# kyle-wedgwood/ArmadilloCUDALinearInterpolation

Measured on AMD Instinct MI355X. Metric: interpolated points/sec (fp64), higher is better.
Workload: dtype f64; 1 GPU; 1D linear interp, 1e+08 random queries on 1e+06-point grid, fp64 (BASELINE configs[1]); queries_per_gpu=100000000, grid_nodes=1000000, table=general, table_mode=0, table_bytes=8000008, entry_point=mi_interp1_f64_dev, query_set=every rank its own set of 100000000 queries

## Files before the change

### armadillocudalinearinterpolation_amd/_lib.py

```python
import ctypes as C
import os

from . import _build

_lib = None


class MiError(RuntimeError):
    def __init__(self, code, msg):
        super().__init__("libmi355interp error %d: %s" % (code, msg))
        self.code = code


class EdmParams(C.Structure):
    _fields_ = [
        ("vth", C.c_float), ("a1", C.c_float), ("a2", C.c_float), ("b1", C.c_float), ("b2", C.c_float),
        ("I", C.c_float), ("L", C.c_float),
        ("newton_tol", C.c_double),
        ("newton_max_iter", C.c_uint32),
        ("n_spikes", C.c_uint32),
        ("time_horizon", C.c_float),
        ("n_grid", C.c_uint32),
        ("n_real", C.c_uint32),
        ("beta_mean", C.c_float),
        ("beta_stddev", C.c_float),
        ("seed", C.c_uint64),
        ("math_mode", C.c_int),
        ("mean_quirk", C.c_int),
        ("max_events", C.c_uint32),
        ("real_offset", C.c_uint32),
        ("dedup_identical", C.c_uint32),
    ]


_vp, _sz, _dbl, _i32, _u32, _f32 = C.c_void_p, C.c_size_t, C.c_double, C.c_int, C.c_uint32, C.c_float
_pp = C.POINTER(C.c_void_p)

SIGNATURES = {
    "mi_abi_version": (_i32, []),
    "mi_debug_pinned_ranges": (_sz, []),
    "mi_debug_sweep_ds_launches": (_sz, []),
    "mi_debug_sweep_ds_launches_base": (_sz, []),
    "mi_debug_interp1_phased_sweep": (_i32, [_vp, _vp, _vp, _vp, _sz, _dbl, _i32, _i32]),
    "mi_debug_each_launches": (_sz, [_i32]),
    "mi_debug_slices2_launches": (_sz, [_i32]),
    "mi_debug_rows1_launches": (_sz, [_i32]),
    "mi_debug_rowpairs_launches": (_sz, [_i32]),
    "mi_debug_nearest_launches": (_sz, [_i32]),
    "mi_debug_nearest_batched_launches": (_sz, [_i32]),
    "mi_debug_grid1_formula": (_i32, [_vp, C.POINTER(_i32), C.POINTER(_i32)]),
    "mi_last_error": (C.c_char_p, [_vp]),
    "mi_ctx_create": (_i32, [_i32, _pp]),
    "mi_ctx_destroy": (_i32, [_vp]),
    "mi_ctx_set_stream": (_i32, [_vp, _vp]),
    "mi_ctx_own_stream": (_i32, [_vp]),
    "mi_ctx_synchronize": (_i32, [_vp]),
    "mi_ctx_set_query_order": (_i32, [_vp, _i32]),
    "mi_ctx_device_info": (_i32, [_vp, C.c_char_p, _sz, C.POINTER(_i32), C.POINTER(_sz)]),
    "mi_timer_create": (_i32, [_vp, _pp]),
    "mi_timer_destroy": (_i32, [_vp]),
    "mi_timer_start": (_i32, [_vp]),
    "mi_timer_stop": (_i32, [_vp]),
    "mi_timer_elapsed_ms": (_i32, [_vp, C.POINTER(_f32)]),
    "mi_grid1_create": (_i32, [_vp, _vp, _vp, _sz, C.c_uint, _pp]),
    "mi_grid1_create_uniform": (_i32, [_vp, _dbl, _dbl, _vp, _sz, C.c_uint, _pp]),
    "mi_grid1_destroy": (_i32, [_vp]),
    "mi_grid1_info": (_i32, [_vp, C.POINTER(_sz), C.POINTER(_i32), C.POINTER(_sz)]),
    "mi_interp1_f64_dev": (_i32, [_vp, _vp, _vp, _vp, _sz, _dbl]),
    "mi_interp1_f64_dev_v2": (_i32, [_vp, _vp, _vp, _vp, _sz, _dbl]),
    "mi_interp1_f64_dev_v2_base": (_i32, [_vp, _vp, _vp, _vp, _sz, _dbl]),
    "mi_interp1_f64_host": (_i32, [_vp, _vp, _vp, _vp, _sz, _dbl]),
    "mi_interp1_f64": (_i32, [_vp, _vp, _vp, _sz, _vp, _vp, _sz, _dbl]),
    "mi_interp1_nearest_f64_dev": (_i32, [_vp, _vp, _vp, _vp, _sz, _dbl]),
    "mi_interp1_nearest_f64_host": (_i32, [_vp, _vp, _vp, _vp, _sz, _dbl]),
    "mi_interp1_nearest_f64": (_i32, [_vp, _vp, _vp, _sz, _vp, _vp, _sz, _dbl]),
    "mi_grid2_create": (_i32, [_vp, _vp, _sz, _vp, _sz, _vp, C.c_uint, _pp]),
    "mi_grid2_create_uniform": (_i32, [_vp, _dbl, _dbl, _sz, _dbl, _dbl, _sz, _vp, C.c_uint, _pp]),
    "mi_grid2_destroy": (_i32, [_vp]),
    "mi_grid2_info": (_i32, [_vp, C.POINTER(_sz)]),
    "mi_interp2_f64_dev": (_i32, [_vp, _vp, _vp, _vp, _vp, _sz, _dbl]),
    "mi_interp2_f64_host": (_i32, [_vp, _vp, _vp, _vp, _vp, _sz, _dbl]),
    "mi_interp2_grid_f64_dev": (_i32, [_vp, _vp, _vp, _sz, _vp, _sz, _vp, _dbl]),
    "mi_interp2_grid_f64_host": (_i32, [_vp, _vp, _vp, _sz, _vp, _sz, _vp, _dbl]),
    "mi_axis1_create": (_i32, [_vp, _vp, _sz, C.c_uint, _pp]),
    "mi_axis1_create_uniform": (_i32, [_vp, _dbl, _dbl, _sz, _pp]),
    "mi_axis1_destroy": (_i32, [_vp]),
    "mi_interp1_cols_f64_dev": (_i32, [_vp, _vp, _vp, _sz, _sz, _vp, _sz, _vp, _sz, _dbl]),
    "mi_interp1_cols_f64_host": (_i32, [_vp, _vp, _vp, _sz, _sz, _vp, _sz, _vp, _sz, _dbl]),
    "mi_interp1_cols_nearest_f64_dev": (_i32, [_vp, _vp, _vp, _sz, _sz, _vp, _sz, _vp, _sz, _dbl]),
    "mi_interp1_pairs_f64_dev": (_i32, [_vp, _vp, _sz, _vp, _sz, _sz, _vp, _sz, _vp, _sz, _vp, _sz, _dbl, _vp]),
    "mi_interp1_pairs_f64_host": (_i32, [_vp, _vp, _sz, _vp, _sz, _sz, _vp, _sz, _vp, _sz, _vp, _sz, _dbl, _vp]),
    "mi_interp1_pairs_nearest_f64_dev": (_i32, [_vp, _vp, _sz, _vp, _sz, _sz, _vp, _sz, _vp, _sz, _vp, _sz, _dbl, _vp]),
    "mi_interp1_each_f64_dev": (_i32, [_vp, _vp, _sz, _vp, _sz, _sz, _vp, _sz, _vp, _sz, _sz, _vp, _sz, _dbl, _vp]),
    "mi_interp1_each_f64_host": (_i32, [_vp, _vp, _sz, _vp, _sz, _sz, _vp, _sz, _vp, _sz, _sz, _vp, _sz, _dbl, _vp]),
    "mi_interp2_slices_f64_dev": (_i32, [_vp, _vp, _vp, _vp, _sz, _sz, _sz, _vp, _sz, _vp, _sz, _vp, _sz, _sz, _dbl]),
    "mi_interp1_rows_f64_dev": (_i32, [_vp, _vp, _vp, _sz, _sz, _vp, _sz, _vp, _sz, _dbl]),
# ... 91 lines not shown
```

### armadillocudalinearinterpolation_amd/csrc/mi_sweep_phase.hip

```cpp
#include <algorithm>
#include <atomic>
#include <cmath>
#include <cstdlib>

#include "mi_interp1_sweep.hpp"

using namespace mi_interp1;

namespace {

constexpr unsigned kTilePeriodNs = 27000;
constexpr unsigned kMaxPeriodNs = 1000000;
constexpr int kPhaseWaitPolls = 4096;
constexpr int kPhasesDefault = 4;

template <int FORMULA, int DEFER>
__global__ __launch_bounds__(kPipeThreads) void interp1_phased_sweep_kernel(G1Dev g, const double* __restrict__ xq,
                                                                            double* __restrict__ yq, size_t ntiles,
                                                                            double extrap, double bscale,
                                                                            const int* __restrict__ order_flag,
                                                                            size_t tail, ProbeArgs probe,
                                                                            unsigned phase_shift, unsigned class_ticks)
{
    constexpr int kVec = kSweepK / 2;
    static_assert(DEFER > 0 && DEFER <= kVec, "DEFER counts result vectors of a lane");
    constexpr int kNow = kVec - DEFER;
    constexpr int kHeld = 2 * DEFER;
    __shared__ double sq[kSweepTile];
    __shared__ unsigned hist[2][kSweepBins];
    __shared__ unsigned gbar[2];
    if (*order_flag != 0) return;
    if (threadIdx.x < 2) gbar[threadIdx.x] = 0;
    const int tid = threadIdx.x & (kPipeGroup - 1);
    const int grp = threadIdx.x >> 9;
    const unsigned nwg = gridDim.x;
    const unsigned phases = 1u << phase_shift;
    const unsigned cls = blockIdx.x & (phases - 1);
    unsigned rank = blockIdx.x >> phase_shift;
    for (unsigned k = 0; k < cls; ++k) rank += nwg > k ? (nwg - k + phases - 1) >> phase_shift : 0;
    const bool last_wg = rank == nwg - 1;
    if (probe.host_mailbox && last_wg && threadIdx.x >= kPipeThreads - 64) order_probe_wave(probe);
    const long nloc = ntiles > rank ? (long)((ntiles - rank + nwg - 1) / nwg) : 0;
    if (cls != 0) {
        const unsigned long long t0 = wall_clock64(), want = (unsigned long long)cls * class_ticks;
        for (int poll = 0; poll < kPhaseWaitPolls && wall_clock64() - t0 < want; ++poll) __builtin_amdgcn_s_sleep(8);
    }
    double q[kSweepK];
    double held[kHeld];
    unsigned sp2[kSweepK / 2];
    auto drop_held = [&]() {
#pragma unroll
        for (int u = 0; u < kHeld; ++u) held[u] = 0.0;
    };
    drop_held();
    const unsigned lane_bytes = (unsigned)tid * (unsigned)sizeof(d2);
    auto vec_at = [&](const double* base, long it, int u) {
        const char* row = reinterpret_cast<const char*>(base + ((size_t)rank + (size_t)it * nwg) * kSweepTile) +
                          (size_t)u * kPipeGroup * sizeof(d2);
        return reinterpret_cast<d2*>(const_cast<char*>(row + lane_bytes));
    };
    auto load_tile = [&](long it) {
#pragma unroll
        for (int u = 0; u < kVec; ++u) {
            const d2 v = stream_load(vec_at(xq, it, u));
            q[2 * u] = v.x;
            q[2 * u + 1] = v.y;
        }
    };
    auto store_now = [&](long it) {
#pragma unroll
        for (int u = 0; u < kNow; ++u) {
            d2 v;
            v.x = q[2 * u];
            v.y = q[2 * u + 1];
            stream_store(v, vec_at(yq, it, u));
        }
    };
    auto store_held = [&](long it) {
        if (it < 0) return;
#pragma unroll
        for (int u = 0; u < DEFER; ++u) {
            d2 v;
            v.x = held[2 * u];
            v.y = held[2 * u + 1];
            stream_store(v, vec_at(yq, it, kNow + u));
        }
    };
    for (int b = threadIdx.x; b < 2 * kSweepBins; b += kPipeThreads) (&hist[0][0])[b] = 0;
    if (grp == 0 && nloc > 0) load_tile(0);
    pipe_barrier();
    unsigned* const myhist = hist[grp];
    unsigned gb_target = 0;
    auto group_barrier = [&]() {
        gb_target += kPipeGroup / 64;
        asm volatile("s_waitcnt lgkmcnt(0)" ::: "memory");
        if ((threadIdx.x & 63) == 0) atomicAdd(&gbar[grp], 1u);
        while (*(lds_vu32*)&gbar[grp] < gb_target) __builtin_amdgcn_s_sleep(2);
        asm volatile("" ::: "memory");
    };
    auto gather_step = [&](long it) {
        const bool act = it >= 0;
        const bool rev = (it & 1) != 0;
        const int stride = rev ? -kPipeGroup : kPipeGroup;
        int first = rev ? kSweepTile - 1 - tid : tid;
        if (act) {
#pragma unroll 1
            for (int iv = 0; iv < 4; ++iv) {
                pipe_gather_rounds<0, FORMULA>(g, sq, first, stride, extrap);
                first += 8 * stride;
            }
        }
        pipe_barrier();
        if (act) {
#pragma unroll
            for (int u = 0; u < kSweepK; u += 2) {
                const double a = sq[sp2[u / 2] & 0xffffu], b = sq[sp2[u / 2] >> 16];
                if (u / 2 < kNow) {
                    q[u] = a;
                    q[u + 1] = b;
                } else {
                    held[u - 2 * kNow] = a;
                    held[u + 1 - 2 * kNow] = b;
                }
                if ((u & 6) == 6) __builtin_amdgcn_sched_barrier(0);
            }
        } else {
#pragma unroll
            for (int u = 0; u < kSweepK; ++u) q[u] = 0.0;
            drop_held();
        }
        pipe_barrier();
        if (act) store_now(it);
        __builtin_amdgcn_sched_barrier(0);
        if (it + 2 < nloc) {
            load_tile(it + 2);
        } else {
#pragma unroll
            for (int u = 0; u < kSweepK; ++u) q[u] = 0.0;
        }
        pipe_barrier();
    };
    auto prep_step = [&](long it) {
        const bool act = it + 1 < nloc;
        store_held(it - 1);
        drop_held();
        unsigned rank2[kSweepK / 2];
#pragma unroll
        for (int u = 0; u < kSweepK / 2; ++u) rank2[u] = 0;
        if (act) {
#pragma unroll
            for (int u = 0; u < kSweepK; u += 2) {
                const unsigned r0 = atomicAdd(&myhist[sweep_bin(q[u], g.xmin, bscale)], 1u);
                const unsigned r1 = atomicAdd(&myhist[sweep_bin(q[u + 1], g.xmin, bscale)], 1u);
                rank2[u / 2] = r0 | (r1 << 16);
                if ((u & 6) == 6) __builtin_amdgcn_sched_barrier(0);
            }
            group_barrier();
            if (tid < 64) sweep_prefix_wave(myhist, tid);
            group_barrier();
#pragma unroll
            for (int u = 0; u < kSweepK; u += 2) {
                double qa = q[u], qb = q[u + 1];
                asm volatile("" : "+v"(qa), "+v"(qb));
                const unsigned p0 = myhist[sweep_bin(qa, g.xmin, bscale)] + (rank2[u / 2] & 0xffffu);
                const unsigned p1 = myhist[sweep_bin(qb, g.xmin, bscale)] + (rank2[u / 2] >> 16);
                sp2[u / 2] = p0 | (p1 << 16);
                if ((u & 6) == 6) __builtin_amdgcn_sched_barrier(0);
            }
        } else {
#pragma unroll
            for (int u = 0; u < kSweepK / 2; ++u) sp2[u] = 0;
        }
        pipe_barrier();
        if (act) {
            for (int b = tid; b < kSweepBins; b += kPipeGroup) myhist[b] = 0;
        }
        pipe_barrier();
        if (act) {
#pragma unroll
            for (int u = 0; u < kSweepK; u += 2) {
                sq[sp2[u / 2] & 0xffffu] = q[u];
                sq[sp2[u / 2] >> 16] = q[u + 1];
                if ((u & 6) == 6) __builtin_amdgcn_sched_barrier(0);
            }
        }
        pipe_barrier();
    };
    if (grp == 0) {
        for (long it = -1;;) {
            prep_step(it);
            if (++it >= nloc) break;
            gather_step(it);
            if (++it >= nloc) break;
        }
    } else {
        for (long it = -1;;) {
            gather_step(it);
            if (++it >= nloc) break;
            prep_step(it);
            if (++it >= nloc) break;
        }
    }
    if (nloc > 0 && grp == (int)((nloc - 1) & 1)) store_held(nloc - 1);
    if (tail && last_wg && grp == 0) pipe_tail<0, FORMULA>(g, xq + ntiles * kSweepTile, yq + ntiles * kSweepTile, tail, tid, extrap);
}

struct PhaseEnv {
    int phases;
    unsigned period_ns;
    bool family_hooks;
};
const PhaseEnv& phase_env()
{
    static const PhaseEnv e = [] {
        PhaseEnv v{kPhasesDefault, kTilePeriodNs, false};
        if (const char* s = getenv("MI_SWEEP_XCD_PHASES")) {
            char* end = nullptr;
            const long p = strtol(s, &end, 10);
            if (end != s && (p == 0 || p == 1 || p == 2 || p == 4 || p == 8)) v.phases = (int)p;
            if (end != s && *end == ':') {
                const long ns = strtol(end + 1, nullptr, 10);
                if (ns >= 0 && ns <= (long)kMaxPeriodNs) v.period_ns = (unsigned)ns;
            }
        }
        v.family_hooks = getenv("MI_SWEEP_MIN_BYTES") || getenv("MI_SWEEP_MIN_TILES_PER_CU") || getenv("MI_SWEEP_VARIANT") ||
                         getenv("MI_SWEEP_DEFER");
        return v;
    }();
    return e;
}

std::atomic<size_t> g_phased_launches{0};

unsigned class_ticks(const mi_ctx* ctx, unsigned period_ns, int phases)
{
    int khz = 0;
    if (hipDeviceGetAttribute(&khz, hipDeviceAttributeWallClockRate, ctx->device) != hipSuccess || khz <= 0) khz = 100000;
    return (unsigned)((double)period_ns * (double)khz * 1e-6 / (double)phases);
}

template <int FORMULA>
mi_status launch_phased(mi_ctx* ctx, const G1Dev& d, const double* xq, double* yq, size_t nq, double extrap, int phases,
                        unsigned period_ns, unsigned max_wg, const ProbeArgs& probe)
{
    const size_t ntiles = nq / kSweepTile, head = ntiles * kSweepTile;
    const double bscale = (double)kSweepBins / (d.xmax - d.xmin);
    const int* flags = reinterpret_cast<const int*>(static_cast<const char*>(ctx->reduce_ws) + mi_ctx::kFlagOffset);
    const unsigned cus = (unsigned)(ctx->compute_units > 0 ? ctx->compute_units : 256);
    const unsigned grid = (unsigned)std::max<size_t>(1, std::min<size_t>(ntiles, (size_t)std::min(cus, max_wg)));
    hipLaunchKernelGGL((interp1_phased_sweep_kernel<FORMULA, kSweepDefer(0)>), dim3(grid), dim3(kPipeThreads), 0, ctx->stream, d,
                       xq, yq, ntiles, extrap, bscale, flags, nq - head, probe, (unsigned)(phases == 8 ? 3 : phases == 4 ? 2 : phases == 2 ? 1 : 0),
                       class_ticks(ctx, period_ns, phases));
    MI_LAUNCH_CHECK(ctx, "interp1 phased region-sweep kernel");
    g_phased_launches.fetch_add(1, std::memory_order_relaxed);
    return MI_OK;
}

mi_status launch_phased_formula(mi_ctx* ctx, const G1Dev& d, const double* xq, double* yq, size_t nq, double extrap, int phases,
                                unsigned period_ns, unsigned max_wg, const ProbeArgs& probe)
{
    if (d.formula == 1) return launch_phased<1>(ctx, d, xq, yq, nq, extrap, phases, period_ns, max_wg, probe);
    if (d.formula == 2) return launch_phased<2>(ctx, d, xq, yq, nq, extrap, phases, period_ns, max_wg, probe);
    if (d.formula == 3) return launch_phased<3>(ctx, d, xq, yq, nq, extrap, phases, period_ns, max_wg, probe);
    return launch_phased<0>(ctx, d, xq, yq, nq, extrap, phases, period_ns, max_wg, probe);
}

bool aligned16(const double* xq, const double* yq)
{
    return ((reinterpret_cast<uintptr_t>(xq) | reinterpret_cast<uintptr_t>(yq)) & 15u) == 0;
}

bool span_ok(const G1Dev& d) { return std::isfinite(d.xmax - d.xmin) && (d.xmax - d.xmin) > 0.0; }

}

extern "C" {

size_t mi_debug_sweep_ds_launches(void)
{
    return mi_debug_sweep_ds_launches_base() + g_phased_launches.load(std::memory_order_relaxed);
}

mi_status mi_interp1_f64_dev_v2(mi_ctx* ctx, const mi_grid1* g, const double* xq, double* yq, size_t nq, double extrap)
{
    const PhaseEnv& e = phase_env();
    bool take = e.phases != 0 && !e.family_hooks && ctx && g && xq && yq && g->mode == 0 && aligned16(xq, yq) &&
                g->table_bytes >= ((size_t)5 << 20) && span_ok(g->d) && ctx->query_order != MI_QUERIES_ORDERED;
    if (take) {
        const size_t cus = (size_t)(ctx->compute_units > 0 ? ctx->compute_units : 256);
        take = nq / kSweepTile >= cus * 16;
    }
    ProbeArgs probe{};
    if (take && ctx->query_order == MI_QUERIES_AUTO) {
        take = *reinterpret_cast<volatile int*>(ctx->probe_host) == 0;
        probe = ProbeArgs{xq, nq, g->d.xmin, (double)kSweepBins / (g->d.xmax - g->d.xmin), nullptr, ctx->probe_host_dev};
    }
    if (!take) return mi_interp1_f64_dev_v2_base(ctx, g, xq, yq, nq, extrap);
    MI_HIP(ctx, hipSetDevice(ctx->device));
    return launch_phased_formula(ctx, g->d, xq, yq, nq, extrap, e.phases, e.period_ns, ~0u, probe);
}

mi_status mi_debug_interp1_phased_sweep(mi_ctx* ctx, const mi_grid1* g, const double* xq, double* yq, size_t nq, double extrap,
                                        int phases, int max_workgroups)
{
    MI_REQUIRE(ctx, ctx && g, "mi_debug_interp1_phased_sweep: NULL context or grid");
    MI_REQUIRE(ctx, g->mode == 0 && span_ok(g->d), "mi_debug_interp1_phased_sweep: closed-form tables (mode 0) of positive finite span only");
    MI_REQUIRE(ctx, phases == 1 || phases == 2 || phases == 4 || phases == 8, "mi_debug_interp1_phased_sweep: phases=%d is not 1, 2, 4 or 8", phases);
    MI_REQUIRE(ctx, max_workgroups >= 1, "mi_debug_interp1_phased_sweep: max_workgroups=%d", max_workgroups);
    if (nq == 0) return MI_OK;
    MI_REQUIRE(ctx, xq && yq && aligned16(xq, yq), "mi_debug_interp1_phased_sweep: pointers must be non-NULL and 16-byte aligned");
    MI_HIP(ctx, hipSetDevice(ctx->device));
    ProbeArgs probe{};
    if (ctx->query_order == MI_QUERIES_AUTO && nq >= 4098)
        probe = ProbeArgs{xq, nq, g->d.xmin, (double)kSweepBins / (g->d.xmax - g->d.xmin), nullptr, ctx->probe_host_dev};
    return launch_phased_formula(ctx, g->d, xq, yq, nq, extrap, phases, phase_env().period_ns, (unsigned)max_workgroups, probe);
}

}
```

### include/mi355_interp.h

```cpp
#ifndef MI355_INTERP_H
#define MI355_INTERP_H

#include <stddef.h>
#include <stdint.h>

#ifdef __cplusplus
extern "C" {
#endif

#define MI355_INTERP_ABI_VERSION 4

typedef int mi_status;
enum {
    MI_OK = 0,
    MI_ERR_INVALID_ARG = 1,
    MI_ERR_GRID = 2,
    MI_ERR_HIP = 3,
    MI_ERR_NOMEM = 4,
    MI_ERR_NO_DEVICE = 5
};

typedef struct mi_ctx mi_ctx;
typedef struct mi_grid1 mi_grid1;
typedef struct mi_grid2 mi_grid2;
typedef struct mi_axis1 mi_axis1;
typedef struct mi_edm mi_edm;
typedef struct mi_timer mi_timer;

mi_status mi_ctx_create(int device, mi_ctx** out);
mi_status mi_ctx_destroy(mi_ctx* ctx);
mi_status mi_ctx_set_stream(mi_ctx* ctx, void* stream);
mi_status mi_ctx_own_stream(mi_ctx* ctx);
mi_status mi_ctx_synchronize(mi_ctx* ctx);
const char* mi_last_error(const mi_ctx* ctx);
int mi_abi_version(void);
size_t mi_debug_pinned_ranges(void);
size_t mi_debug_sweep_ds_launches(void);
size_t mi_debug_sweep_ds_launches_base(void);
size_t mi_debug_each_launches(int form);
size_t mi_debug_slices2_launches(int form);
size_t mi_debug_rows1_launches(int form);
size_t mi_debug_rowpairs_launches(int form);
size_t mi_debug_nearest_launches(int form);
size_t mi_debug_nearest_batched_launches(int form);
mi_status mi_debug_grid1_formula(const mi_grid1* g, int* formula, int* pin_last);
#define MI_QUERIES_AUTO    0
#define MI_QUERIES_RANDOM  1
#define MI_QUERIES_ORDERED 2
mi_status mi_ctx_set_query_order(mi_ctx* ctx, int order);
mi_status mi_ctx_device_info(mi_ctx* ctx, char* name, size_t name_len, int* compute_units,
                             size_t* hbm_bytes);

mi_status mi_timer_create(mi_ctx* ctx, mi_timer** out);
mi_status mi_timer_destroy(mi_timer* t);
mi_status mi_timer_start(mi_timer* t);
mi_status mi_timer_stop(mi_timer* t);
mi_status mi_timer_elapsed_ms(mi_timer* t, float* ms);

#define MI_GRID_SANITISE     0x1u
#define MI_GRID_DEVICE_PTRS  0x2u
mi_status mi_grid1_create(mi_ctx* ctx, const double* x, const double* y, size_t n,
                          unsigned flags, mi_grid1** out);
mi_status mi_grid1_create_uniform(mi_ctx* ctx, double x0, double dx, const double* y, size_t n,
                                  unsigned flags, mi_grid1** out);
mi_status mi_grid1_destroy(mi_grid1* g);
mi_status mi_grid1_info(const mi_grid1* g, size_t* n_nodes, int* mode, size_t* table_bytes);

mi_status mi_interp1_f64_dev(mi_ctx* ctx, const mi_grid1* g, const double* xq_dev, double* yq_dev,
                             size_t nq, double extrap_val);
mi_status mi_interp1_f64_dev_v2(mi_ctx* ctx, const mi_grid1* g, const double* xq_dev, double* yq_dev,
                                size_t nq, double extrap_val);
mi_status mi_interp1_f64_dev_v2_base(mi_ctx* ctx, const mi_grid1* g, const double* xq_dev, double* yq_dev,
                                     size_t nq, double extrap_val);
mi_status mi_debug_interp1_phased_sweep(mi_ctx* ctx, const mi_grid1* g, const double* xq_dev, double* yq_dev,
                                        size_t nq, double extrap_val, int phases, int max_workgroups);
mi_status mi_interp1_f64_host(mi_ctx* ctx, const mi_grid1* g, const double* xq, double* yq,
                              size_t nq, double extrap_val);
mi_status mi_interp1_f64(mi_ctx* ctx, const double* x, const double* y, size_t n, const double* xq,
                         double* yq, size_t nq, double extrap_val);

mi_status mi_interp1_nearest_f64_dev(mi_ctx* ctx, const mi_grid1* g, const double* xq_dev, double* yq_dev,
                                     size_t nq, double extrap_val);
mi_status mi_interp1_nearest_f64_host(mi_ctx* ctx, const mi_grid1* g, const double* xq, double* yq,
                                      size_t nq, double extrap_val);
mi_status mi_interp1_nearest_f64(mi_ctx* ctx, const double* x, const double* y, size_t n, const double* xq,
                                 double* yq, size_t nq, double extrap_val);

#define MI_GRID2_COMPACT 0x4u
mi_status mi_grid2_create(mi_ctx* ctx, const double* x, size_t nx, const double* y, size_t ny,
                          const double* z, unsigned flags, mi_grid2** out);
mi_status mi_grid2_create_uniform(mi_ctx* ctx, double x0, double dx, size_t nx, double y0, double dy,
                                  size_t ny, const double* z, unsigned flags, mi_grid2** out);
mi_status mi_grid2_destroy(mi_grid2* g);
mi_status mi_grid2_info(const mi_grid2* g, size_t* table_bytes);
mi_status mi_interp2_f64_dev(mi_ctx* ctx, const mi_grid2* g, const double* xq_dev,
                             const double* yq_dev, double* zq_dev, size_t nq, double extrap_val);
mi_status mi_interp2_f64_host(mi_ctx* ctx, const mi_grid2* g, const double* xq, const double* yq,
                              double* zq, size_t nq, double extrap_val);
mi_status mi_interp2_grid_f64_dev(mi_ctx* ctx, const mi_grid2* g, const double* xi_dev, size_t nxi,
                                  const double* yi_dev, size_t nyi, double* zi_dev, double extrap_val);
mi_status mi_interp2_grid_f64_host(mi_ctx* ctx, const mi_grid2* g, const double* xi, size_t nxi,
                                   const double* yi, size_t nyi, double* zi, double extrap_val);

mi_status mi_axis1_create(mi_ctx* ctx, const double* x, size_t n, unsigned flags, mi_axis1** out);
mi_status mi_axis1_create_uniform(mi_ctx* ctx, double x0, double dx, size_t n, mi_axis1** out);
mi_status mi_axis1_destroy(mi_axis1* axis);
mi_status mi_interp1_cols_f64_dev(mi_ctx* ctx, const mi_axis1* axis, const double* y_dev, size_t ldy, size_t ncols,
                                  const double* xi_dev, size_t nxi, double* yi_dev, size_t ldyi, double extrap_val);
mi_status mi_interp1_cols_f64_host(mi_ctx* ctx, const mi_axis1* axis, const double* y, size_t ldy, size_t ncols,
                                   const double* xi, size_t nxi, double* yi, size_t ldyi, double extrap_val);
mi_status mi_interp1_cols_nearest_f64_dev(mi_ctx* ctx, const mi_axis1* axis, const double* y_dev, size_t ldy, size_t ncols,
                                          const double* xi_dev, size_t nxi, double* yi_dev, size_t ldyi, double extrap_val);

mi_status mi_interp1_pairs_f64_dev(mi_ctx* ctx, const double* x_dev, size_t ldx, const double* y_dev, size_t ldy, size_t n,
                                   const uint32_t* len_dev, size_t ncols, const double* xi_dev, size_t nxi,
                                   double* yi_dev, size_t ldyi, double extrap_val, uint32_t* col_ok_dev);
mi_status mi_interp1_pairs_f64_host(mi_ctx* ctx, const double* x, size_t ldx, const double* y, size_t ldy, size_t n,
                                    const uint32_t* len, size_t ncols, const double* xi, size_t nxi, double* yi,
                                    size_t ldyi, double extrap_val, uint32_t* col_ok);
mi_status mi_interp1_pairs_nearest_f64_dev(mi_ctx* ctx, const double* x_dev, size_t ldx, const double* y_dev, size_t ldy,
                                           size_t n, const uint32_t* len_dev, size_t ncols, const double* xi_dev,
                                           size_t nxi, double* yi_dev, size_t ldyi, double extrap_val,
                                           uint32_t* col_ok_dev);

mi_status mi_interp1_each_f64_dev(mi_ctx* ctx, const double* x_dev, size_t ldx, const double* y_dev, size_t ldy, size_t n,
                                  const uint32_t* len_dev, size_t ncols, const double* xi_dev, size_t ldxi, size_t nxi,
                                  double* yi_dev, size_t ldyi, double extrap_val, uint32_t* col_ok_dev);
mi_status mi_interp1_each_f64_host(mi_ctx* ctx, const double* x, size_t ldx, const double* y, size_t ldy, size_t n,
// ... 134 lines not shown
```

Measured before the change: 164.5 billion points/s.

## Stagger phase classes with partial first tiles instead of clock waits

Splits the phased sweep's work into quarter-tile units and gives each phase class a first tile of a different size (1..4 units). This staggers when workgroups hit the memory-heavy phases without spinning on the wall clock. A partition function balances the remaining units across workgroups and handles partial last tiles. It also adds optional timestamp recording and debug entry points, at the cost of more index arithmetic and 32-bit query counting limits.

```diff
diff --git a/armadillocudalinearinterpolation_amd/_lib.py b/armadillocudalinearinterpolation_amd/_lib.py
--- a/armadillocudalinearinterpolation_amd/_lib.py
+++ b/armadillocudalinearinterpolation_amd/_lib.py
@@ -42,6 +42,8 @@
     "mi_debug_sweep_ds_launches": (_sz, []),
     "mi_debug_sweep_ds_launches_base": (_sz, []),
     "mi_debug_interp1_phased_sweep": (_i32, [_vp, _vp, _vp, _vp, _sz, _dbl, _i32, _i32]),
+    "mi_debug_interp1_phased_sweep_ex": (_i32, [_vp, _vp, _vp, _vp, _sz, _dbl, _i32, _i32, _u32, _vp, _u32]),
+    "mi_debug_sweep_partition": (_i32, [_sz, _u32, _i32, _u32, _u32] + [C.POINTER(_u32)] * 3 + [C.POINTER(_sz)] * 6),
     "mi_debug_each_launches": (_sz, [_i32]),
     "mi_debug_slices2_launches": (_sz, [_i32]),
     "mi_debug_rows1_launches": (_sz, [_i32]),
diff --git a/armadillocudalinearinterpolation_amd/csrc/mi_sweep_partition.hpp b/armadillocudalinearinterpolation_amd/csrc/mi_sweep_partition.hpp
--- /dev/null
+++ b/armadillocudalinearinterpolation_amd/csrc/mi_sweep_partition.hpp
@@ -0,0 +1,115 @@
+#pragma once
+#include <cstddef>
+
+namespace mi_sweep {
+
+constexpr unsigned kUnitQueries = 4096;
+constexpr unsigned kTileUnits = 4;
+constexpr unsigned kMaxPhases = 8;
+
+template <class I>
+struct PartitionT {
+    unsigned ntiles;
+    unsigned first_units;
+    unsigned last_units;
+    I work;
+    I first_start;
+    I mid_origin;
+    I mid_step;
+    I pen_start;
+    I last_start;
+};
+using Partition = PartitionT<size_t>;
+
+__host__ __device__ inline unsigned pack_first_units(unsigned decimal, unsigned P)
+{
+    if (P == 0 || P > kMaxPhases) return 0;
+    unsigned nibbles = 0;
+    for (unsigned k = P; k-- > 0;) {
+        const unsigned digit = decimal % 10u;
+        decimal /= 10u;
+        if (digit < 1 || digit > kTileUnits) return 0;
+        nibbles |= digit << (4 * k);
+    }
+    return decimal == 0 ? nibbles : 0;
+}
+__host__ __device__ inline unsigned first_units_of(unsigned nibbles, unsigned k) { return (nibbles >> (4 * k)) & 15u; }
+
+__host__ __device__ inline unsigned class_size(unsigned nwg, unsigned P, unsigned k) { return nwg > k ? (nwg - k + P - 1) / P : 0; }
+
+namespace detail {
+
+template <class I>
+struct Sums {
+    I first, row1, row2;
+};
+
+template <class I>
+__host__ __device__ inline I min_sz(I a, I b) { return a < b ? a : b; }
+
+template <class I>
+__host__ __device__ inline Sums<I> sums_below(unsigned upto, unsigned nwg, unsigned P, unsigned fu, I w, unsigned rem, I R)
+{
+    Sums<I> s{0, 0, 0};
+    unsigned a = 0;
+    for (unsigned k = 0; k < P; ++k) {
+        const unsigned b = a + class_size(nwg, P, k), hi = b < upto ? b : upto;
+        if (hi > a) {
+            const unsigned n1 = rem > a ? (rem < hi ? rem - a : hi - a) : 0;
+            for (unsigned more = 0; more < 2; ++more) {
+                const I cnt = more ? n1 : hi - a - n1;
+                if (cnt == 0) continue;
+                const I share = w + more, f = min_sz<I>(first_units_of(fu, k), share), left = share - f - kTileUnits * R;
+                s.first += cnt * f;
+                s.row1 += cnt * min_sz<I>(left, kTileUnits);
+                s.row2 += cnt * (left > kTileUnits ? left - kTileUnits : 0);
+            }
+        }
+        a = b;
+    }
+    return s;
+}
+
+}
+
+template <class I>
+__host__ __device__ inline PartitionT<I> sweep_partition(I U, unsigned nwg, unsigned P, unsigned first_units, unsigned rank)
+{
+    PartitionT<I> p{};
+    if (nwg == 0 || rank >= nwg || P == 0 || P > kMaxPhases) return p;
+    const I w = U / nwg;
+    const unsigned rem = (unsigned)(U % nwg);
+    I least = ~(I)0;
+    unsigned a = 0, cls = 0;
+    for (unsigned k = 0; k < P; ++k) {
+        const unsigned b = a + class_size(nwg, P, k);
+        if (b > a) {
+            if (rem > a) least = detail::min_sz<I>(least, w + 1 - detail::min_sz<I>(first_units_of(first_units, k), w + 1));
+            if (rem < b) least = detail::min_sz<I>(least, w - detail::min_sz<I>(first_units_of(first_units, k), w));
+            if (rank >= a && rank < b) cls = k;
+        }
+        a = b;
+    }
+    const I R = least / kTileUnits;
+    const detail::Sums<I> all = detail::sums_below<I>(nwg, nwg, P, first_units, w, rem, R);
+    const detail::Sums<I> low = detail::sums_below<I>(rank, nwg, P, first_units, w, rem, R);
+    p.work = w + (rank < rem ? 1 : 0);
+    const I f = detail::min_sz<I>(first_units_of(first_units, cls), p.work), left = p.work - f - kTileUnits * R;
+    const unsigned t1 = (unsigned)detail::min_sz<I>(left, kTileUnits), t2 = left > kTileUnits ? (unsigned)(left - kTileUnits) : 0;
+    p.first_units = (unsigned)f;
+    p.first_start = low.first;
+    p.mid_origin = all.first + (I)kTileUnits * rank;
+    p.mid_step = (I)kTileUnits * nwg;
+    if (f == 0) return p;
+    const I row1 = all.first + p.mid_step * R + low.row1, row2 = all.first + p.mid_step * R + all.row1 + low.row2;
+    const I ntiles = 1 + R + (t1 ? 1 : 0) + (t2 ? 1 : 0);
+    p.ntiles = (unsigned)ntiles;
+    auto start_of = [&](I i) { return i == 0 ? p.first_start : i <= R ? p.mid_origin + (i - 1) * p.mid_step : i == R + 1 ? row1 : row2; };
+    auto units_of = [&](I i) { return i == 0 ? (unsigned)f : i <= R ? kTileUnits : i == R + 1 ? t1 : t2; };
+    p.last_start = start_of(ntiles - 1);
+    p.last_units = units_of(ntiles - 1);
+    p.pen_start = ntiles >= 2 ? start_of(ntiles - 2) : p.first_start;
+    return p;
+}
+
+}
diff --git a/armadillocudalinearinterpolation_amd/csrc/mi_sweep_phase.hip b/armadillocudalinearinterpolation_amd/csrc/mi_sweep_phase.hip
--- a/armadillocudalinearinterpolation_amd/csrc/mi_sweep_phase.hip
+++ b/armadillocudalinearinterpolation_amd/csrc/mi_sweep_phase.hip
@@ -2,8 +2,10 @@
 #include <atomic>
 #include <cmath>
 #include <cstdlib>
+#include <type_traits>
 
 #include "mi_interp1_sweep.hpp"
+#include "mi_sweep_partition.hpp"
 
 using namespace mi_interp1;
 
@@ -13,23 +15,47 @@
 constexpr unsigned kMaxPeriodNs = 1000000;
 constexpr int kPhaseWaitPolls = 4096;
 constexpr int kPhasesDefault = 4;
-
-template <int FORMULA, int DEFER>
+constexpr size_t kMaxQueries = (size_t)1 << 43;
+constexpr unsigned kFirstUnits4 = 1234;
+constexpr unsigned kFirstUnits2 = 0;
+
+template <int J>
+using unit_c = std::integral_constant<int, J>;
+template <class Body, class Skip>
+__device__ __forceinline__ void for_units(unsigned nu, Body&& body, Skip&& skip)
+{
+    if (nu > 0) body(unit_c<0>{}); else skip(unit_c<0>{});
+    if (nu > 1) body(unit_c<1>{}); else skip(unit_c<1>{});
+    if (nu > 2) body(unit_c<2>{}); else skip(unit_c<2>{});
+    if (nu > 3) body(unit_c<3>{}); else skip(unit_c<3>{});
+}
+
+template <int FORMULA, int DEFER, bool STAMP>
 __global__ __launch_bounds__(kPipeThreads) void interp1_phased_sweep_kernel(G1Dev g, const double* __restrict__ xq,
-                                                                            double* __restrict__ yq, size_t ntiles,
+                                                                            double* __restrict__ yq, size_t nq,
                                                                             double extrap, double bscale,
                                                                             const int* __restrict__ order_flag,
-                                                                            size_t tail, ProbeArgs probe,
-                                                                            unsigned phase_shift, unsigned class_ticks)
+                                                                            ProbeArgs probe, unsigned phase_shift,
+                                                                            unsigned class_ticks, unsigned first_units,
+                                                                            unsigned long long* __restrict__ stamps,
+                                                                            unsigned stamp_cap)
 {
     constexpr int kVec = kSweepK / 2;
+    constexpr int kUnitVec = kVec / (int)mi_sweep::kTileUnits;
     static_assert(DEFER > 0 && DEFER <= kVec, "DEFER counts result vectors of a lane");
+    static_assert(kSweepTile == (int)(mi_sweep::kTileUnits * mi_sweep::kUnitQueries) && kUnitVec == 4, "a unit is a quarter of a tile");
     constexpr int kNow = kVec - DEFER;
     constexpr int kHeld = 2 * DEFER;
     __shared__ double sq[kSweepTile];
     __shared__ unsigned hist[2][kSweepBins];
     __shared__ unsigned gbar[2];
     if (*order_flag != 0) return;
+    auto stamp = [&](unsigned slot) __attribute__((always_inline)) {
+        if constexpr (STAMP) {
+            if (slot < stamp_cap) stamps[(size_t)blockIdx.x * stamp_cap + slot] = wall_clock64();
+        }
+    };
+    if (threadIdx.x == 0) stamp(0);
     if (threadIdx.x < 2) gbar[threadIdx.x] = 0;
     const int tid = threadIdx.x & (kPipeGroup - 1);
     const int grp = threadIdx.x >> 9;
@@ -39,91 +65,155 @@
     unsigned rank = blockIdx.x >> phase_shift;
     for (unsigned k = 0; k < cls; ++k) rank += nwg > k ? (nwg - k + phases - 1) >> phase_shift : 0;
     const bool last_wg = rank == nwg - 1;
-    if (probe.host_mailbox && last_wg && threadIdx.x >= kPipeThreads - 64) order_probe_wave(probe);
-    const long nloc = ntiles > rank ? (long)((ntiles - rank + nwg - 1) / nwg) : 0;
-    if (cls != 0) {
+    auto scalar = [](unsigned v) __attribute__((always_inline)) { return (unsigned)__builtin_amdgcn_readfirstlane((int)v); };
+    const unsigned step = mi_sweep::kTileUnits * nwg;
+    unsigned ntl, org, nus = mi_sweep::kTileUnits | (mi_sweep::kTileUnits << 4), d_first = 0, d_pen = 0, d_last = 0;
+    if (first_units == 0) {
+        const unsigned ntiles = (unsigned)(nq / kSweepTile);
+        ntl = scalar(ntiles > rank ? (ntiles - rank + nwg - 1) / nwg : 0);
+        org = mi_sweep::kTileUnits * rank + step;
+    } else {
+        const mi_sweep::PartitionT<unsigned> part =
+            mi_sweep::sweep_partition<unsigned>((unsigned)(nq / mi_sweep::kUnitQueries), nwg, phases, first_units, rank);
+        ntl = scalar(part.ntiles);
+        nus = scalar(part.first_units | (part.last_units << 4));
+        org = scalar(part.mid_origin);
+        d_first = scalar(part.first_start - (part.mid_origin - step));
+        if (part.ntiles >= 2) d_last = scalar(part.last_start - (part.mid_origin + (part.ntiles - 2) * step));
+        if (part.ntiles >= 3) d_pen = scalar(part.pen_start - (part.mid_origin + (part.ntiles - 3) * step));
+    }
+    const long nloc = (long)ntl;
+    const unsigned k_org = org, k_nus = nus, k_first = d_first, k_pen = d_pen, k_last = d_last;
+    auto tile_units = [scalar, ntl, k_nus](long it) __attribute__((always_inline)) {
+        const unsigned i = scalar((unsigned)it);
+        return i == 0 ? k_nus & 15u : i == ntl - 1 ? k_nus >> 4 : mi_sweep::kTileUnits;
+    };
+    auto tile_at = [scalar, ntl, step, k_org, k_first, k_pen, k_last](long it) __attribute__((always_inline)) {
+        const unsigned i = scalar((unsigned)it);
+        const unsigned fix = i == 0 ? k_first : i == ntl - 1 ? k_last : i == ntl - 2 ? k_pen : 0u;
+        return k_org + (i - 1u) * step + fix;
+    };
+    if (cls != 0 && class_ticks != 0) {
         const unsigned long long t0 = wall_clock64(), want = (unsigned long long)cls * class_ticks;
         for (int poll = 0; poll < kPhaseWaitPolls && wall_clock64() - t0 < want; ++poll) __builtin_amdgcn_s_sleep(8);
     }
     double q[kSweepK];
     double held[kHeld];
     unsigned sp2[kSweepK / 2];
-    auto drop_held = [&]() {
+    auto drop_held = [&]() __attribute__((always_inline)) {
 #pragma unroll
         for (int u = 0; u < kHeld; ++u) held[u] = 0.0;
     };
     drop_held();
     const unsigned lane_bytes = (unsigned)tid * (unsigned)sizeof(d2);
-    auto vec_at = [&](const double* base, long it, int u) {
-        const char* row = reinterpret_cast<const char*>(base + ((size_t)rank + (size_t)it * nwg) * kSweepTile) +
-                          (size_t)u * kPipeGroup * sizeof(d2);
-        return reinterpret_cast<d2*>(const_cast<char*>(row + lane_bytes));
-    };
-    auto load_tile = [&](long it) {
-#pragma unroll
-        for (int u = 0; u < kVec; ++u) {
-            const d2 v = stream_load(vec_at(xq, it, u));
-            q[2 * u] = v.x;
-            q[2 * u + 1] = v.y;
-        }
-    };
-    auto store_now = [&](long it) {
-#pragma unroll
-        for (int u = 0; u < kNow; ++u) {
-            d2 v;
-            v.x = q[2 * u];
-            v.y = q[2 * u + 1];
-            stream_store(v, vec_at(yq, it, u));
-        }
-    };
-    auto store_held = [&](long it) {
+    auto vec_at = [&](const double* base, long it, int u) __attribute__((always_inline)) {
+        const char* row = reinterpret_cast<const char*>(base + (size_t)tile_at(it) * mi_sweep::kUnitQueries);
+        asm("" : "+s"(row));
+        return reinterpret_cast<d2*>(const_cast<char*>(row + (size_t)u * kPipeGroup * sizeof(d2) + lane_bytes));
+    };
+    auto load_tile = [&](long it) __attribute__((always_inline)) {
+        for_units(tile_units(it),
+                  [&](auto j) __attribute__((always_inline)) {
+                      constexpr int J = decltype(j)::value;
+#pragma unroll
+                      for (int u = kUnitVec * J; u < kUnitVec * (J + 1); ++u) {
+                          const d2 v = stream_load(vec_at(xq, it, u));
+                          q[2 * u] = v.x;
+                          q[2 * u + 1] = v.y;
+                      }
+                  },
+                  [&](auto j) __attribute__((always_inline)) {
+                      constexpr int J = decltype(j)::value;
+#pragma unroll
+                      for (int u = 2 * kUnitVec * J; u < 2 * kUnitVec * (J + 1); ++u) q[u] = 0.0;
+                  });
+    };
+    auto store_now = [&](long it) __attribute__((always_inline)) {
+        for_units(tile_units(it),
+                  [&](auto j) __attribute__((always_inline)) {
+                      constexpr int J = decltype(j)::value;
+#pragma unroll
+                      for (int u = kUnitVec * J; u < kUnitVec * (J + 1); ++u) {
+                          if (u < kNow) {
+                              d2 v;
+                              v.x = q[2 * u];
+                              v.y = q[2 * u + 1];
+                              stream_store(v, vec_at(yq, it, u));
+                          }
+                      }
+                  },
+                  [&](auto) __attribute__((always_inline)) {});
+    };
+    auto store_held = [&](long it) __attribute__((always_inline)) {
         if (it < 0) return;
-#pragma unroll
-        for (int u = 0; u < DEFER; ++u) {
-            d2 v;
-            v.x = held[2 * u];
-            v.y = held[2 * u + 1];
-            stream_store(v, vec_at(yq, it, kNow + u));
-        }
+        for_units(tile_units(it),
+                  [&](auto j) __attribute__((always_inline)) {
+                      constexpr int J = decltype(j)::value;
+#pragma unroll
+                      for (int u = kUnitVec * J; u < kUnitVec * (J + 1); ++u) {
+                          if (u >= kNow) {
+                              d2 v;
+                              v.x = held[2 * (u - kNow)];
+                              v.y = held[2 * (u - kNow) + 1];
+                              stream_store(v, vec_at(yq, it, u));
+                          }
+                      }
+                  },
+                  [&](auto) __attribute__((always_inline)) {});
     };
     for (int b = threadIdx.x; b < 2 * kSweepBins; b += kPipeThreads) (&hist[0][0])[b] = 0;
     if (grp == 0 && nloc > 0) load_tile(0);
     pipe_barrier();
+    if (probe.host_mailbox && last_wg && threadIdx.x >= kPipeThreads - 64) order_probe_wave(probe);
     unsigned* const myhist = hist[grp];
     unsigned gb_target = 0;
-    auto group_barrier = [&]() {
+    auto group_barrier = [&]() __attribute__((always_inline)) {
         gb_target += kPipeGroup / 64;
         asm volatile("s_waitcnt lgkmcnt(0)" ::: "memory");
         if ((threadIdx.x & 63) == 0) atomicAdd(&gbar[grp], 1u);
         while (*(lds_vu32*)&gbar[grp] < gb_target) __builtin_amdgcn_s_sleep(2);
         asm volatile("" ::: "memory");
     };
-    auto gather_step = [&](long it) {
+    auto gather_step = [&](long it) __attribute__((always_inline)) {
         const bool act = it >= 0;
+        const unsigned nu = act ? tile_units(it) : 0;
         const bool rev = (it & 1) != 0;
         const int stride = rev ? -kPipeGroup : kPipeGroup;
-        int first = rev ? kSweepTile - 1 - tid : tid;
+        int first = rev ? (int)(nu * mi_sweep::kUnitQueries) - 1 - tid : tid;
         if (act) {
+            if (tid == 0) stamp(1u + (unsigned)it);
 #pragma unroll 1
-            for (int iv = 0; iv < 4; ++iv) {
+            for (int iv = 0; iv < (int)nu; ++iv) {
                 pipe_gather_rounds<0, FORMULA>(g, sq, first, stride, extrap);
                 first += 8 * stride;
             }
         }
         pipe_barrier();
         if (act) {
-#pragma unroll
-            for (int u = 0; u < kSweepK; u += 2) {
-                const double a = sq[sp2[u / 2] & 0xffffu], b = sq[sp2[u / 2] >> 16];
-                if (u / 2 < kNow) {
-                    q[u] = a;
-                    q[u + 1] = b;
-                } else {
-                    held[u - 2 * kNow] = a;
-                    held[u + 1 - 2 * kNow] = b;
-                }
-                if ((u & 6) == 6) __builtin_amdgcn_sched_barrier(0);
-            }
+            for_units(nu,
+                      [&](auto j) __attribute__((always_inline)) {
+                      constexpr int J = decltype(j)::value;
+#pragma unroll
+                          for (int u = 8 * J; u < 8 * (J + 1); u += 2) {
+                              const double a = sq[sp2[u / 2] & 0xffffu], b = sq[sp2[u / 2] >> 16];
+                              if (u / 2 < kNow) {
+                                  q[u] = a;
+                                  q[u + 1] = b;
+                              } else {
+                                  held[u - 2 * kNow] = a;
+                                  held[u + 1 - 2 * kNow] = b;
+                              }
+                          }
+                          __builtin_amdgcn_sched_barrier(0);
+                      },
+                      [&](auto j) __attribute__((always_inline)) {
+                      constexpr int J = decltype(j)::value;
+#pragma unroll
+                          for (int u = 8 * J; u < 8 * (J + 1); ++u) {
+                              if (u / 2 < kNow) q[u] = 0.0;
+                              else held[u - 2 * kNow] = 0.0;
+                          }
+                      });
         } else {
 #pragma unroll
             for (int u = 0; u < kSweepK; ++u) q[u] = 0.0;
@@ -140,33 +230,48 @@
         }
         pipe_barrier();
     };
-    auto prep_step = [&](long it) {
+    auto prep_step = [&](long it) __attribute__((always_inline)) {
         const bool act = it + 1 < nloc;
+        const unsigned nu = act ? tile_units(it + 1) : 0;
         store_held(it - 1);
         drop_held();
         unsigned rank2[kSweepK / 2];
 #pragma unroll
         for (int u = 0; u < kSweepK / 2; ++u) rank2[u] = 0;
         if (act) {
-#pragma unroll
-            for (int u = 0; u < kSweepK; u += 2) {
-                const unsigned r0 = atomicAdd(&myhist[sweep_bin(q[u], g.xmin, bscale)], 1u);
-                const unsigned r1 = atomicAdd(&myhist[sweep_bin(q[u + 1], g.xmin, bscale)], 1u);
-                rank2[u / 2] = r0 | (r1 << 16);
-                if ((u & 6) == 6) __builtin_amdgcn_sched_barrier(0);
-            }
+            for_units(nu,
+                      [&](auto j) __attribute__((always_inline)) {
+                      constexpr int J = decltype(j)::value;
+#pragma unroll
+                          for (int u = 8 * J; u < 8 * (J + 1); u += 2) {
+                              const unsigned r0 = atomicAdd(&myhist[sweep_bin(q[u], g.xmin, bscale)], 1u);
+                              const unsigned r1 = atomicAdd(&myhist[sweep_bin(q[u + 1], g.xmin, bscale)], 1u);
+                              rank2[u / 2] = r0 | (r1 << 16);
+                          }
+                          __builtin_amdgcn_sched_barrier(0);
+                      },
+                      [&](auto) __attribute__((always_inline)) {});
             group_barrier();
             if (tid < 64) sweep_prefix_wave(myhist, tid);
             group_barrier();
-#pragma unroll
-            for (int u = 0; u < kSweepK; u += 2) {
-                double qa = q[u], qb = q[u + 1];
-                asm volatile("" : "+v"(qa), "+v"(qb));
-                const unsigned p0 = myhist[sweep_bin(qa, g.xmin, bscale)] + (rank2[u / 2] & 0xffffu);
-                const unsigned p1 = myhist[sweep_bin(qb, g.xmin, bscale)] + (rank2[u / 2] >> 16);
-                sp2[u / 2] = p0 | (p1 << 16);
-                if ((u & 6) == 6) __builtin_amdgcn_sched_barrier(0);
-            }
+            for_units(nu,
+                      [&](auto j) __attribute__((always_inline)) {
+                      constexpr int J = decltype(j)::value;
+#pragma unroll
+                          for (int u = 8 * J; u < 8 * (J + 1); u += 2) {
+                              double qa = q[u], qb = q[u + 1];
+                              asm volatile("" : "+v"(qa), "+v"(qb));
+                              const unsigned p0 = myhist[sweep_bin(qa, g.xmin, bscale)] + (rank2[u / 2] & 0xffffu);
+                              const unsigned p1 = myhist[sweep_bin(qb, g.xmin, bscale)] + (rank2[u / 2] >> 16);
+                              sp2[u / 2] = p0 | (p1 << 16);
+                          }
+                          __builtin_amdgcn_sched_barrier(0);
+                      },
+                      [&](auto j) __attribute__((always_inline)) {
+                      constexpr int J = decltype(j)::value;
+#pragma unroll
+                          for (int u = 4 * J; u < 4 * (J + 1); ++u) sp2[u] = 0;
+                      });
         } else {
 #pragma unroll
             for (int u = 0; u < kSweepK / 2; ++u) sp2[u] = 0;
@@ -177,12 +282,17 @@
         }
         pipe_barrier();
         if (act) {
-#pragma unroll
-            for (int u = 0; u < kSweepK; u += 2) {
-                sq[sp2[u / 2] & 0xffffu] = q[u];
-                sq[sp2[u / 2] >> 16] = q[u + 1];
-                if ((u & 6) == 6) __builtin_amdgcn_sched_barrier(0);
-            }
+            for_units(nu,
+                      [&](auto j) __attribute__((always_inline)) {
+                      constexpr int J = decltype(j)::value;
+#pragma unroll
+                          for (int u = 8 * J; u < 8 * (J + 1); u += 2) {
+                              sq[sp2[u / 2] & 0xffffu] = q[u];
+                              sq[sp2[u / 2] >> 16] = q[u + 1];
+                          }
+                          __builtin_amdgcn_sched_barrier(0);
+                      },
+                      [&](auto) __attribute__((always_inline)) {});
         }
         pipe_barrier();
     };
@@ -202,25 +312,50 @@
         }
     }
     if (nloc > 0 && grp == (int)((nloc - 1) & 1)) store_held(nloc - 1);
-    if (tail && last_wg && grp == 0) pipe_tail<0, FORMULA>(g, xq + ntiles * kSweepTile, yq + ntiles * kSweepTile, tail, tid, extrap);
-}
-
-struct PhaseEnv {
+    const size_t tail = nq & (size_t)((first_units ? mi_sweep::kUnitQueries : (unsigned)kSweepTile) - 1u), whole = nq - tail;
+    if (tail && last_wg && grp == 0) pipe_tail<0, FORMULA>(g, xq + whole, yq + whole, tail, tid, extrap);
+    if (threadIdx.x == 0) stamp(1u + (unsigned)nloc);
+}
+
+struct PhaseForm {
     int phases;
     unsigned period_ns;
+    unsigned first_units;
+};
+
+constexpr unsigned first_units_default(int phases) { return phases == 4 ? kFirstUnits4 : phases == 2 ? kFirstUnits2 : 0; }
+
+struct PhaseEnv {
+    PhaseForm form;
     bool family_hooks;
 };
+PhaseForm clock_form(int phases, unsigned period_ns) { return PhaseForm{phases, period_ns, 0}; }
+PhaseForm shipped_form(int phases)
+{
+    const unsigned packed = phases < 8 ? mi_sweep::pack_first_units(first_units_default(phases), (unsigned)phases) : 0;
+    return packed ? PhaseForm{phases, 0, packed} : clock_form(phases, kTilePeriodNs);
+}
 const PhaseEnv& phase_env()
 {
     static const PhaseEnv e = [] {
-        PhaseEnv v{kPhasesDefault, kTilePeriodNs, false};
+        PhaseEnv v{shipped_form(kPhasesDefault), false};
         if (const char* s = getenv("MI_SWEEP_XCD_PHASES")) {
             char* end = nullptr;
             const long p = strtol(s, &end, 10);
-            if (end != s && (p == 0 || p == 1 || p == 2 || p == 4 || p == 8)) v.phases = (int)p;
+            int phases = kPhasesDefault;
+            if (end != s && (p == 0 || p == 1 || p == 2 || p == 4 || p == 8)) phases = (int)p;
+            v.form = shipped_form(phases);
             if (end != s && *end == ':') {
-                const long ns = strtol(end + 1, nullptr, 10);
-                if (ns >= 0 && ns <= (long)kMaxPeriodNs) v.period_ns = (unsigned)ns;
+                char* end2 = nullptr;
+                const long ns = strtol(end + 1, &end2, 10);
+                const bool ns_ok = end2 != end + 1 && ns >= 0 && ns <= (long)kMaxPeriodNs;
+                unsigned packed = 0;
+                if (*end2 == ':' && phases >= 1 && phases < 8) {
+                    const long units = strtol(end2 + 1, nullptr, 10);
+                    if (units > 0 && units <= 44444444) packed = mi_sweep::pack_first_units((unsigned)units, (unsigned)phases);
+                }
+                if (packed) v.form = PhaseForm{phases, ns_ok ? (unsigned)ns : 0u, packed};
+                else if (ns_ok && (ns > 0 || v.form.first_units == 0)) v.form = clock_form(phases, (unsigned)ns);
             }
         }
         v.family_hooks = getenv("MI_SWEEP_MIN_BYTES") || getenv("MI_SWEEP_MIN_TILES_PER_CU") || getenv("MI_SWEEP_VARIANT") ||
@@ -234,35 +369,46 @@
 
 unsigned class_ticks(const mi_ctx* ctx, unsigned period_ns, int phases)
 {
+    if (period_ns == 0) return 0;
     int khz = 0;
     if (hipDeviceGetAttribute(&khz, hipDeviceAttributeWallClockRate, ctx->device) != hipSuccess || khz <= 0) khz = 100000;
     return (unsigned)((double)period_ns * (double)khz * 1e-6 / (double)phases);
 }
 
+struct StampArgs {
+    unsigned long long* buf;
+    unsigned cap;
+};
+
 template <int FORMULA>
-mi_status launch_phased(mi_ctx* ctx, const G1Dev& d, const double* xq, double* yq, size_t nq, double extrap, int phases,
-                        unsigned period_ns, unsigned max_wg, const ProbeArgs& probe)
-{
-    const size_t ntiles = nq / kSweepTile, head = ntiles * kSweepTile;
+mi_status launch_phased(mi_ctx* ctx, const G1Dev& d, const double* xq, double* yq, size_t nq, double extrap, const PhaseForm& f,
+                        unsigned max_wg, const ProbeArgs& probe, const StampArgs& st)
+{
+    const size_t pieces = f.first_units ? nq / mi_sweep::kUnitQueries : nq / kSweepTile;
     const double bscale = (double)kSweepBins / (d.xmax - d.xmin);
     const int* flags = reinterpret_cast<const int*>(static_cast<const char*>(ctx->reduce_ws) + mi_ctx::kFlagOffset);
     const unsigned cus = (unsigned)(ctx->compute_units > 0 ? ctx->compute_units : 256);
-    const unsigned grid = (unsigned)std::max<size_t>(1, std::min<size_t>(ntiles, (size_t)std::min(cus, max_wg)));
-    hipLaunchKernelGGL((interp1_phased_sweep_kernel<FORMULA, kSweepDefer(0)>), dim3(grid), dim3(kPipeThreads), 0, ctx->stream, d,
-                       xq, yq, ntiles, extrap, bscale, flags, nq - head, probe, (unsigned)(phases == 8 ? 3 : phases == 4 ? 2 : phases == 2 ? 1 : 0),
-                       class_ticks(ctx, period_ns, phases));
+    const unsigned grid = (unsigned)std::max<size_t>(1, std::min<size_t>(pieces, (size_t)std::min(cus, max_wg)));
+    const unsigned shift = (unsigned)(f.phases == 8 ? 3 : f.phases == 4 ? 2 : f.phases == 2 ? 1 : 0);
+    const unsigned ticks = class_ticks(ctx, f.period_ns, f.phases);
+    if (st.buf)
+        hipLaunchKernelGGL((interp1_phased_sweep_kernel<FORMULA, kSweepDefer(0), true>), dim3(grid), dim3(kPipeThreads), 0, ctx->stream, d,
+                           xq, yq, nq, extrap, bscale, flags, probe, shift, ticks, f.first_units, st.buf, st.cap);
+    else
+        hipLaunchKernelGGL((interp1_phased_sweep_kernel<FORMULA, kSweepDefer(0), false>), dim3(grid), dim3(kPipeThreads), 0, ctx->stream, d,
+                           xq, yq, nq, extrap, bscale, flags, probe, shift, ticks, f.first_units, (unsigned long long*)nullptr, 0u);
     MI_LAUNCH_CHECK(ctx, "interp1 phased region-sweep kernel");
     g_phased_launches.fetch_add(1, std::memory_order_relaxed);
     return MI_OK;
 }
 
-mi_status launch_phased_formula(mi_ctx* ctx, const G1Dev& d, const double* xq, double* yq, size_t nq, double extrap, int phases,
-                                unsigned period_ns, unsigned max_wg, const ProbeArgs& probe)
-{
-    if (d.formula == 1) return launch_phased<1>(ctx, d, xq, yq, nq, extrap, phases, period_ns, max_wg, probe);
-    if (d.formula == 2) return launch_phased<2>(ctx, d, xq, yq, nq, extrap, phases, period_ns, max_wg, probe);
-    if (d.formula == 3) return launch_phased<3>(ctx, d, xq, yq, nq, extrap, phases, period_ns, max_wg, probe);
-    return launch_phased<0>(ctx, d, xq, yq, nq, extrap, phases, period_ns, max_wg, probe);
+mi_status launch_phased_formula(mi_ctx* ctx, const G1Dev& d, const double* xq, double* yq, size_t nq, double extrap, const PhaseForm& f,
+                                unsigned max_wg, const ProbeArgs& probe, const StampArgs& st = StampArgs{nullptr, 0})
+{
+    if (d.formula == 1) return launch_phased<1>(ctx, d, xq, yq, nq, extrap, f, max_wg, probe, st);
+    if (d.formula == 2) return launch_phased<2>(ctx, d, xq, yq, nq, extrap, f, max_wg, probe, st);
+    if (d.formula == 3) return launch_phased<3>(ctx, d, xq, yq, nq, extrap, f, max_wg, probe, st);
+    return launch_phased<0>(ctx, d, xq, yq, nq, extrap, f, max_wg, probe, st);
 }
 
 bool aligned16(const double* xq, const double* yq)
@@ -284,11 +430,11 @@
 mi_status mi_interp1_f64_dev_v2(mi_ctx* ctx, const mi_grid1* g, const double* xq, double* yq, size_t nq, double extrap)
 {
     const PhaseEnv& e = phase_env();
-    bool take = e.phases != 0 && !e.family_hooks && ctx && g && xq && yq && g->mode == 0 && aligned16(xq, yq) &&
+    bool take = e.form.phases != 0 && !e.family_hooks && ctx && g && xq && yq && g->mode == 0 && aligned16(xq, yq) &&
                 g->table_bytes >= ((size_t)5 << 20) && span_ok(g->d) && ctx->query_order != MI_QUERIES_ORDERED;
     if (take) {
         const size_t cus = (size_t)(ctx->compute_units > 0 ? ctx->compute_units : 256);
-        take = nq / kSweepTile >= cus * 16;
+        take = nq / kSweepTile >= cus * 16 && nq <= kMaxQueries;
     }
     ProbeArgs probe{};
     if (take && ctx->query_order == MI_QUERIES_AUTO) {
@@ -297,7 +443,7 @@
     }
     if (!take) return mi_interp1_f64_dev_v2_base(ctx, g, xq, yq, nq, extrap);
     MI_HIP(ctx, hipSetDevice(ctx->device));
-    return launch_phased_formula(ctx, g->d, xq, yq, nq, extrap, e.phases, e.period_ns, ~0u, probe);
+    return launch_phased_formula(ctx, g->d, xq, yq, nq, extrap, e.form, ~0u, probe);
 }
 
 mi_status mi_debug_interp1_phased_sweep(mi_ctx* ctx, const mi_grid1* g, const double* xq, double* yq, size_t nq, double extrap,
@@ -308,12 +454,59 @@
     MI_REQUIRE(ctx, phases == 1 || phases == 2 || phases == 4 || phases == 8, "mi_debug_interp1_phased_sweep: phases=%d is not 1, 2, 4 or 8", phases);
     MI_REQUIRE(ctx, max_workgroups >= 1, "mi_debug_interp1_phased_sweep: max_workgroups=%d", max_workgroups);
     if (nq == 0) return MI_OK;
+    MI_REQUIRE(ctx, nq <= kMaxQueries, "mi_debug_interp1_phased_sweep: nq=%zu is more than the kernel counts in 32 bits", nq);
     MI_REQUIRE(ctx, xq && yq && aligned16(xq, yq), "mi_debug_interp1_phased_sweep: pointers must be non-NULL and 16-byte aligned");
     MI_HIP(ctx, hipSetDevice(ctx->device));
     ProbeArgs probe{};
     if (ctx->query_order == MI_QUERIES_AUTO && nq >= 4098)
         probe = ProbeArgs{xq, nq, g->d.xmin, (double)kSweepBins / (g->d.xmax - g->d.xmin), nullptr, ctx->probe_host_dev};
-    return launch_phased_formula(ctx, g->d, xq, yq, nq, extrap, phases, phase_env().period_ns, (unsigned)max_workgroups, probe);
-}
-
-}
+    const PhaseForm& env = phase_env().form;
+    return launch_phased_formula(ctx, g->d, xq, yq, nq, extrap, clock_form(phases, env.first_units ? kTilePeriodNs : env.period_ns),
+                                 (unsigned)max_workgroups, probe);
+}
+
+mi_status mi_debug_interp1_phased_sweep_ex(mi_ctx* ctx, const mi_grid1* g, const double* xq, double* yq, size_t nq, double extrap,
+                                           int phases, int max_workgroups, unsigned first_units, unsigned long long* stamps,
+                                           unsigned stamp_cap)
+{
+    MI_REQUIRE(ctx, ctx && g, "mi_debug_interp1_phased_sweep_ex: NULL context or grid");
+    MI_REQUIRE(ctx, g->mode == 0 && span_ok(g->d), "mi_debug_interp1_phased_sweep_ex: closed-form tables (mode 0) of positive finite span only");
+    MI_REQUIRE(ctx, phases == 1 || phases == 2 || phases == 4 || phases == 8, "mi_debug_interp1_phased_sweep_ex: phases=%d is not 1, 2, 4 or 8", phases);
+    MI_REQUIRE(ctx, max_workgroups >= 1, "mi_debug_interp1_phased_sweep_ex: max_workgroups=%d", max_workgroups);
+    const unsigned packed = first_units && phases < 8 ? mi_sweep::pack_first_units(first_units, (unsigned)phases) : 0;
+    MI_REQUIRE(ctx, first_units == 0 || packed != 0, "mi_debug_interp1_phased_sweep_ex: first_units=%u is not %d digits in 1..4 (and phases 1, 2 or 4)",
+               first_units, phases);
+    MI_REQUIRE(ctx, stamps == nullptr || stamp_cap >= 2, "mi_debug_interp1_phased_sweep_ex: stamp_cap=%u with a stamp buffer", stamp_cap);
+    if (nq == 0) return MI_OK;
+    MI_REQUIRE(ctx, nq <= kMaxQueries, "mi_debug_interp1_phased_sweep_ex: nq=%zu is more than the kernel counts in 32 bits", nq);
+    MI_REQUIRE(ctx, xq && yq && aligned16(xq, yq), "mi_debug_interp1_phased_sweep_ex: pointers must be non-NULL and 16-byte aligned");
+    MI_HIP(ctx, hipSetDevice(ctx->device));
+    ProbeArgs probe{};
+    if (ctx->query_order == MI_QUERIES_AUTO && nq >= 4098)
+        probe = ProbeArgs{xq, nq, g->d.xmin, (double)kSweepBins / (g->d.xmax - g->d.xmin), nullptr, ctx->probe_host_dev};
+    const PhaseForm& env = phase_env().form;
+    const PhaseForm f = packed ? PhaseForm{phases, 0, packed} : clock_form(phases, env.first_units ? kTilePeriodNs : env.period_ns);
+    return launch_phased_formula(ctx, g->d, xq, yq, nq, extrap, f, (unsigned)max_workgroups, probe, StampArgs{stamps, stamp_cap});
+}
+
+mi_status mi_debug_sweep_partition(size_t nq, unsigned nwg, int phases, unsigned first_units, unsigned rank, unsigned* ntiles,
+                             unsigned* first_tile_units, unsigned* last_tile_units, size_t* work, size_t* first_start,
+                             size_t* mid_origin, size_t* mid_step, size_t* pen_start, size_t* last_start)
+{
+    if (!(phases == 1 || phases == 2 || phases == 4) || nwg == 0 || rank >= nwg) return MI_ERR_INVALID_ARG;
+    const unsigned packed = mi_sweep::pack_first_units(first_units, (unsigned)phases);
+    if (!packed) return MI_ERR_INVALID_ARG;
+    const mi_sweep::Partition p = mi_sweep::sweep_partition<size_t>(nq / mi_sweep::kUnitQueries, nwg, (unsigned)phases, packed, rank);
+    if (ntiles) *ntiles = p.ntiles;
+    if (first_tile_units) *first_tile_units = p.first_units;
+    if (last_tile_units) *last_tile_units = p.last_units;
+    if (work) *work = p.work;
+    if (first_start) *first_start = p.first_start;
+    if (mid_origin) *mid_origin = p.mid_origin;
+    if (mid_step) *mid_step = p.mid_step;
+    if (pen_start) *pen_start = p.pen_start;
+    if (last_start) *last_start = p.last_start;
+    return MI_OK;
+}
+
+}
diff --git a/include/mi355_interp.h b/include/mi355_interp.h
--- a/include/mi355_interp.h
+++ b/include/mi355_interp.h
@@ -74,6 +74,13 @@
                                      size_t nq, double extrap_val);
 mi_status mi_debug_interp1_phased_sweep(mi_ctx* ctx, const mi_grid1* g, const double* xq_dev, double* yq_dev,
                                         size_t nq, double extrap_val, int phases, int max_workgroups);
+mi_status mi_debug_interp1_phased_sweep_ex(mi_ctx* ctx, const mi_grid1* g, const double* xq_dev, double* yq_dev,
+                                           size_t nq, double extrap_val, int phases, int max_workgroups,
+                                           unsigned first_units, unsigned long long* stamps_dev, unsigned stamp_cap);
+mi_status mi_debug_sweep_partition(size_t nq, unsigned nwg, int phases, unsigned first_units, unsigned rank,
+                                   unsigned* ntiles, unsigned* first_tile_units, unsigned* last_tile_units, size_t* work,
+                                   size_t* first_start, size_t* mid_origin, size_t* mid_step, size_t* pen_start,
+                                   size_t* last_start);
 mi_status mi_interp1_f64_host(mi_ctx* ctx, const mi_grid1* g, const double* xq, double* yq,
                               size_t nq, double extrap_val);
 mi_status mi_interp1_f64(mi_ctx* ctx, const double* x, const double* y, size_t n, const double* xq,
```

Measured after the change: 169.0 billion points/s (median of 6 runs). +2.7%, better.
